# Fytex/Shafa-CD

Hardware: AMD Instinct MI355X
Metric: GiB/s Shannon-Fano encode+decode, 64 MiB blocks, 1/2/4/8 GPUs; bit-exact (higher is better)
Workload: dtype u8

## Files before the change

### shafa-cd_amd/csrc/sf_decode.hip

```cpp
#include <type_traits>
#include "common.hpp"
#include "internal.hpp"

#include <atomic>
#include <mutex>
#include <thread>

#include <algorithm>

#include <stdlib.h>

#include "sfd_common.hpp"
#include "sfd_dp.hpp"
#include "sfd_generic.hpp"

namespace {

typedef __attribute__((address_space(3))) u32 lds_u32;
typedef __attribute__((address_space(3))) u16 lds_u16;
typedef __attribute__((address_space(3))) u8 lds_u8;
template <int LONG> constexpr u32 spec_emask() { return LONG == 2 ? 31u : 15u; }

constexpr int SC_PHW = 16;
constexpr int SC_M = 4;
// ... 446 lines not shown
constexpr int SL_SW = 16;
constexpr int SL_ROW = SL_SW + 1;
constexpr int SL_STRIPS = DEC_THREADS + 1;
constexpr int SL_LDS_DATA = (SL_STRIPS * SL_ROW + 3) / 4 * 16;
constexpr int SL_MISC = DEC_THREADS + 16 + 32;

struct SlWin {
    u32 lo, hi, wa;
    __device__ __forceinline__ void init() { wa = 0xFFFFFFFFu; hi = lo = 0; }
    __device__ __forceinline__ u32 at(u32 q)
    {
        const u32 a = (q >> 3) & ~3u;
        if (a != wa) {
            const lds_u32 *pa = (const lds_u32 *)(size_t)a;
            lo = pa[0];
            hi = pa[1];
            wa = a;
        }
        return __builtin_amdgcn_alignbit(hi, lo, q);
    }
};

template <int LONG>
__device__ __forceinline__ void sl_walk(const lds_u8 *tab, const u16 *lt, const u32 KW, u32 &q, const u32 qe, const int qlimit, u32 &cnt, SlWin &sw)
{
    const u32 mask = (1u << KW) - 1u;
    auto long_len = [&](const u32 qq) -> u32 {
        const u32 win = __builtin_bitreverse32(sw.at(qq));
        const u32 l = (LONG == 1 ? long_code(lt, win) : long_code32(lt, win)) >> 8;
        return l ? l : 1u;
    };
    const u32 nlook = KW <= 10 ? 3u : 2u;
    while (q + nlook * KW <= qe && (int)(q + nlook * KW) <= qlimit) {
        const u32 w = sw.at(q);
        u32 sum = 0, e = 0;
        for (u32 i = 0; i < nlook; ++i) {
            e = tab[(w >> (sum & 31u)) & mask];
            sum += e;
        }
        q += sum & 31u;
        cnt += sum >> 5;
        if (LONG && __builtin_expect((e & 31u) == 0u, 0)) {
            const u32 l = long_len(q);
            if ((int)(q + l) > qlimit) { q = qe + spec_emask<LONG>(); return; }
            q += l;
            ++cnt;
        }
    }
    const lds_u8 *len0 = tab + (1u << KW);
    while (q < qe) {
        u32 l0 = len0[sw.at(q) & mask];
        if (LONG && __builtin_expect(l0 == 0u, 0)) l0 = long_len(q);
        if ((int)(q + l0) > qlimit) { q = qe + spec_emask<LONG>(); break; }
        q += l0;
        ++cnt;
    }
}

template <bool HAVE_OLD, int LONG>
__device__ __forceinline__ void sl_strip(const lds_u8 *tab, const u16 *lt, const u32 KW, const u32 qrow, const int qlimit, const u32 ent0,
                                         u32 (&ent)[2], u32 (&cnt)[2], u32 &exit_)
{
    u32 q = qrow + ent0;
    SlWin sw;
    sw.init();
#pragma unroll
    for (int k = 0; k < 2; ++k) {
        const u32 r = q - (qrow + 256u * k);
        if (HAVE_OLD && k > 0 && r == ent[k]) return;
        ent[k] = r;
        u32 c = 0;
        sl_walk<LONG>(tab, lt, KW, q, qrow + 256u * (k + 1), qlimit, c, sw);
        cnt[k] = c;
    }
    exit_ = (q - (qrow + 512u)) & spec_emask<LONG>();
}

template <int LONG>
__device__ __forceinline__ u32 sl_region(u8 *smem, const DecBlk &blk, const u32 tile0, const u32 e0_forced, u8 *__restrict__ chunk_entry,
                                         u16 *__restrict__ chunk_cnt, u32 *__restrict__ tile_cnt, u8 *__restrict__ tile_guess,
                                         u8 *__restrict__ tile_exit, const u32 tab_bytes)
{
    const u64 start = (u64)tile0 * DTILE;
    const u64 left = blk.in_n > start ? blk.in_n - start : 0;
    const size_t gt0 = (size_t)blk.tile_base + tile0;
    const u32 ntl = blk.n_tiles - tile0 < (u32)SC_WTILES ? blk.n_tiles - tile0 : (u32)SC_WTILES;
    u32 *data = (u32 *)smem;
    const u32 tab_off = SL_LDS_DATA;
    u8 *ex = smem + SL_LDS_DATA + tab_bytes;
    const u32 tid = threadIdx.x, lane = tid & 63, wv = tid >> 6;
    const u32 KW = blk.KW;
    const u16 *lt = (const u16 *)(smem + SL_LDS_DATA + tab_bytes + SL_MISC);
    {
        const long long base = (long long)start - 4 * SL_SW;
        constexpr u32 UNITS = (u32)(SL_STRIPS * SL_SW / 4 + 1), NIT = (UNITS + DEC_THREADS - 1) / DEC_THREADS;
        uint4 v[NIT];
#pragma unroll
        for (u32 it = 0; it < NIT; ++it) {
            const u32 i = tid + it * DEC_THREADS;
            const long long off = base + (long long)i * 16;
            v[it] = make_uint4(0, 0, 0, 0);
            if (i < UNITS && off >= 0 && (u64)off + 16 <= blk.in_n) v[it] = gload<uint4>(blk.in + off);
        }
#pragma unroll
        for (u32 it = 0; it < NIT; ++it) {
            const u32 i = tid + it * DEC_THREADS;
            if (i >= UNITS) break;
            const long long off = base + (long long)i * 16;
            u32 w[4] = {v[it].x, v[it].y, v[it].z, v[it].w};
            if (off >= 0 && (u64)off < blk.in_n && (u64)off + 16 > blk.in_n) {
                const int nv = (int)(blk.in_n - (u64)off);
#pragma unroll
                for (int q = 0; q < 16; ++q)
                    if (q < nv) w[q >> 2] |= (u32)gload<u8>(blk.in + off + q) << (8 * (q & 3));
            }
            const u32 f = 4 * i, at = f + f / SL_SW;
            const u32 w0 = rev_bytes(w[0]);
            if (f % SL_SW == 0 && f > 0) data[at - 1] = w0;
            if (i < UNITS - 1) {
                data[at] = w0;
                data[at + 1] = rev_bytes(w[1]);
                data[at + 2] = rev_bytes(w[2]);
                data[at + 3] = rev_bytes(w[3]);
            }
        }
    }
    __syncthreads();
    const int limit = (int)(left * 8) - (int)(512u * tid);
    const u32 qrow = 8u * ((4u * SL_ROW) * (tid + 1));
    const int qlimit = (int)qrow + limit;
    const lds_u8 *tab = (const lds_u8 *)(size_t)tab_off;
    u32 ent[2] = {0, 0}, cnt[2] = {0, 0}, exit_ = 0;
    {
        u32 e0;
        if (tid == 0) e0 = e0_forced;
        else {
            const u32 qe = qrow;
            u32 q = qe - 256u, dummy = 0;
            SlWin sw;
            sw.init();
            sl_walk<LONG>(tab, lt, KW, q, qe, qlimit, dummy, sw);
            e0 = (q - qe) & spec_emask<LONG>();
        }
        sl_strip<false, LONG>(tab, lt, KW, qrow, qlimit, e0, ent, cnt, exit_);
    }
    ex[tid] = (u8)exit_;
    __syncthreads();
    bool bad = false;
    u32 *const wsum = (u32 *)(ex + DEC_THREADS), *const flags = wsum + 4;
    u32 turn = 0;
    for (int round = 0; round < 4; ++round) {
        bad = tid > 0 && ent[0] != (u32)ex[tid - 1];
        if (!wg_any(bad, flags, turn)) break;
        if (bad) sl_strip<true, LONG>(tab, lt, KW, qrow, qlimit, (u32)ex[tid - 1], ent, cnt, exit_);
        __syncthreads();
        ex[tid] = (u8)exit_;
        __syncthreads();
        bad = tid > 0 && ent[0] != (u32)ex[tid - 1];
    }
    if (wg_any(bad, flags, turn)) {
        if (tid == 0) __hip_atomic_store(blk.run_dp, 1u, __ATOMIC_RELAXED, __HIP_MEMORY_SCOPE_AGENT);
    }
    const u32 my_tile = tid / 128u;
    const u32 wtot = dpp_scan_add(cnt[0] + cnt[1]);
    if (lane == 63) wsum[wv] = wtot;
    __syncthreads();
    if (my_tile < ntl) {
        const size_t c0 = gt0 * DEC_THREADS + (size_t)tid * 2;
        gstore<u16>(chunk_entry + c0, (u16)((ent[0] & 0xFFu) | (ent[1] << 8)));
        gstore<u32>(chunk_cnt + c0, cnt[0] | (cnt[1] << 16));
        const u32 in_tile = tid & 127u;
        if (in_tile == 0) {
            tile_cnt[gt0 + my_tile] = wsum[2 * my_tile] + wsum[2 * my_tile + 1];
            tile_guess[gt0 + my_tile] = (u8)ent[0];
        }
        if (in_tile == 127u) tile_exit[gt0 + my_tile] = (u8)exit_;
    }
    const u32 unit_exit = ex[ntl * 128u - 1u];
    __syncthreads();
    return unit_exit;
}

constexpr u32 SF_CHUNKS = 8;

constexpr u32 SF_LINKS = 2 * DEC_THREADS;
template <int LONG>
__device__ __forceinline__ void sf_links(u8 *smem, const DecBlk &blk, const u32 t_begin, const u32 t_end, u8 *__restrict__ chunk_entry,
                                         u16 *__restrict__ chunk_cnt, u32 *__restrict__ tile_cnt, u8 *__restrict__ tile_guess,
                                         const u8 *__restrict__ tile_exit, const u32 tab_bytes, const u32 long_bytes)
{
    const u32 tid = threadIdx.x, KW = blk.KW, mask = (1u << KW) - 1u;
    const u16 *lt = (const u16 *)(smem + tab_bytes + 48);
    const u8 *len0 = smem + (1u << KW);
    const u64 end_bit = blk.in_n * 8;
    u32 turn = 0;
    u32 xs[SF_LINKS / DEC_THREADS];
    bool any_bad = false;
#pragma unroll
    for (u32 i = 0; i < SF_LINKS / DEC_THREADS; ++i) {
        const u32 t = t_begin + tid + i * DEC_THREADS;
        xs[i] = 0xFFFFFFFFu;
        if (t < t_end) {
            const size_t gt = (size_t)blk.tile_base + t;
            const u32 x = tile_exit[gt - 1];
            if (tile_guess[gt] != x) { xs[i] = x; any_bad = true; }
        }
    }
    if (!wg_any(any_bad, (u32 *)(smem + tab_bytes), turn)) return;
    __syncthreads();
    fill_lds16((void *)smem, (const void *)blk.cnt3, 2u << KW);
    if (LONG) {
        const u16 *src = LONG == 1 ? blk.longtab : blk.long32;
        if (src) fill_lds16((void *)lt, src, long_bytes);
        else if (tid == 0) *(u16 *)lt = 0;
    }
    bool failed = false;
    volatile u32 *const gave_up = (volatile u32 *)(smem + tab_bytes + 32);
    if (tid == 0) *gave_up = 0;
    __syncthreads();
#pragma unroll 1
    for (u32 i = 0; i < SF_LINKS / DEC_THREADS; ++i) {
        if (*gave_up) break;
        const u32 x = xs[i];
        if (x == 0xFFFFFFFFu) continue;
        const u32 t = t_begin + tid + i * DEC_THREADS;
        const size_t gt = (size_t)blk.tile_base + t;
        const u64 tile_bit0 = (u64)t * DTILE * 8;
        if (x >= spec_emask<LONG>() || tile_bit0 + (u64)(SF_CHUNKS + 1) * CH_BITS + 64 > end_bit) { failed = true; *gave_up = 1; continue; }
        u32 q = x, wi = 0xFFFFFFFFu, lo = 0, hi = 0;
        auto window = [&](const u32 qq) -> u32 {
            const u32 i = qq >> 5;
            if (i != wi) {
                const u8 *p = blk.in + (u64)t * DTILE + 4u * i;
                lo = rev_bytes(gload<u32>(p));
                hi = rev_bytes(gload<u32>(p + 4));
                wi = i;
            }
            return __builtin_amdgcn_alignbit(hi, lo, qq);
        };
        int delta = 0;
        bool merged = false;
        const size_t c0 = gt * DEC_THREADS;
        for (u32 c = 0; c < SF_CHUNKS; ++c) {
            const u32 qe = CH_BITS * (c + 1);
            u32 cnt = 0;
            while (q < qe) {
                const u32 w = window(q);
                u32 l = len0[w & mask];
                if (LONG && l == 0u) {
                    const u32 win = __builtin_bitreverse32(w);
                    l = (LONG == 1 ? long_code(lt, win) : long_code32(lt, win)) >> 8;
                    if (!l) l = 1u;
                }
                q += l;
                ++cnt;
            }
            delta += (int)cnt - (int)chunk_cnt[c0 + c];
            chunk_cnt[c0 + c] = (u16)cnt;
            const u32 e = q - qe;
            if (e == (u32)chunk_entry[c0 + c + 1]) { merged = true; break; }
            chunk_entry[c0 + c + 1] = (u8)e;
        }
        if (!merged) { failed = true; *gave_up = 1; continue; }
        chunk_entry[c0] = (u8)x;
        tile_guess[gt] = (u8)x;
        tile_cnt[gt] = (u32)((int)tile_cnt[gt] + delta);
    }
    if (wg_any(failed, (u32 *)(smem + tab_bytes), turn) && tid == 0)
        __hip_atomic_store(blk.run_dp, 1u, __ATOMIC_RELAXED, __HIP_MEMORY_SCOPE_AGENT);
}

template <int LONG>
__global__ __launch_bounds__(DEC_THREADS) void sfd_ends(const DecBlk *__restrict__ blks, u8 *__restrict__ chunk_entry,
                                                        u16 *__restrict__ chunk_cnt, u32 *__restrict__ tile_cnt,
                                                        u8 *__restrict__ tile_guess, u8 *__restrict__ tile_exit, u32 tab_bytes, u32 long_bytes)
{
    extern __shared__ __attribute__((aligned(16))) u8 smem[];
    const DecBlk blk = blks[blockIdx.y];
    if (!blk.n_tiles || !blk.run_dp || __hip_atomic_load(blk.run_dp, __ATOMIC_RELAXED, __HIP_MEMORY_SCOPE_AGENT) != 0) return;
    if (lds_addr(smem) != 0) __builtin_trap();
    const u32 units = (blk.n_tiles + SC_WTILES - 1) / SC_WTILES;
    u32 first_end = units - 1;
    if (units >= 2 && blk.in_n - (u64)(units - 2) * SC_WTILES * DTILE < (u64)64 * SC_SB + 4) first_end = units - 2;
    if (blockIdx.x > 0) {
        const u32 t_end = first_end * SC_WTILES, t_begin = 1u + (blockIdx.x - 1u) * SF_LINKS;
        if (t_begin < t_end)
            sf_links<LONG>(smem, blk, t_begin, t_end, chunk_entry, chunk_cnt, tile_cnt, tile_guess, tile_exit, tab_bytes, long_bytes);
        return;
    }
    fill_lds16((void *)(smem + SL_LDS_DATA), (const void *)blk.cnt3, 2u << blk.KW);
    if (LONG) {
        u16 *lt = (u16 *)(smem + SL_LDS_DATA + tab_bytes + SL_MISC);
        const u16 *src = LONG == 1 ? blk.longtab : blk.long32;
        if (src) fill_lds16((void *)lt, src, long_bytes);
        else if (threadIdx.x == 0) *lt = 0;
    }
    __syncthreads();
    u32 e0 = first_end ? (u32)tile_exit[(size_t)blk.tile_base + first_end * SC_WTILES - 1] : 0u;
    for (u32 u = first_end; u < units; ++u)
        e0 = sl_region<LONG>(smem, blk, u * SC_WTILES, e0, chunk_entry, chunk_cnt, tile_cnt, tile_guess, tile_exit, tab_bytes);
}

constexpr int ws_row(bool esc) { return CH_BYTES / 4 + (esc ? 3 : 2); }
constexpr int ws_rows_bytes(bool esc)
{
    return 16 + (DEC_THREADS * ws_row(esc) + (esc ? 0 : DEC_THREADS / 16)) * 4;
}
constexpr int WS_MISC = 32;
typedef unsigned int u32x3_t __attribute__((ext_vector_type(3)));
constexpr u32 WS_NST = 4, WS_DROP = 0x7FFFFFF0u;
constexpr int WS_RSRC_FLAGS = 0x00020000, WS_AUX_NT = 2;

__device__ __forceinline__ void ws_walk1(const u32 tab_off, const u32 mask2, const u32 xa, u32 q2, const u32 q2end, u32 want,
                                         const bool by_pos)
{
    auto window2 = [&]() -> u32 {
        const lds_u32 *pa = (const lds_u32 *)(size_t)((q2 >> 3) & ~3u);
        return __builtin_amdgcn_alignbit(pa[1], pa[0], q2);
    };
    auto look = [&](const u32 w) -> u32 { return *(const lds_u16 *)(size_t)(tab_off + (w & mask2)); };
    auto image_or = [](const u32 at, const u32 v) {
        __hip_atomic_fetch_or((lds_u32 *)(size_t)at, v, __ATOMIC_RELAXED, __HIP_MEMORY_SCOPE_WORKGROUP);
    };
    if (by_pos) {
        constexpr u32 N = 3, F = 4, WPG = F * N / 4;
        const u32 s = (0u - xa) & 3u;
        u32 ptr = ((xa + 3u) & ~3u) - 4u;
        u32 L = 0, Lp = 0, Ep = 0;
        auto group = [&](auto first_group) -> bool {
            constexpr bool FIRST = decltype(first_group)::value;
            u32 x0 = 0, x1 = 0, ub = 0;
#pragma unroll
            for (u32 f = 0; f < F; ++f) {
                if (!((int)q2 < (int)q2end)) {
                    if (f == 0) {
                        if (!FIRST) {
                            image_or(ptr + 4u * (WPG - 1u), Ep);
                            image_or(ptr + 4u * WPG, __builtin_amdgcn_alignbyte(0u, Lp, s));
                        }
                    } else {
                        const u32 at = ptr + 4u * (f * N >> 2);
                        image_or(at, __builtin_amdgcn_alignbyte(L, Lp, s));
                        image_or(at + 4u, __builtin_amdgcn_alignbyte(0u, L, s));
                    }
                    return false;
                }
                if (f == 0 && !FIRST) {
                    *(lds_u32 *)(size_t)(ptr + 4u * (WPG - 1u)) = Ep;
                    ptr += 4u * WPG;
                }
                u32 w;
                if ((f & 1u) == 0) {
                    const lds_u32 *pa = (const lds_u32 *)(size_t)((q2 >> 3) & ~3u);
                    const u32 w0 = pa[0], w1 = pa[1], w2 = pa[2];
                    w = x0 = __builtin_amdgcn_alignbit(w1, w0, q2);
                    x1 = __builtin_amdgcn_alignbit(w2, w1, q2);
                } else
                    w = __builtin_amdgcn_alignbit(x1, x0, ub);
                u32 ua = 0;
#pragma unroll
                for (u32 i = 0; i < N; ++i) {
                    const u32 k = f * N + i, b = k & 3u;
                    const u32 e = look(w >> ua);
                    ua += e >> 8;
                    L = __builtin_amdgcn_perm(e, L, b == 0 ? 0x0C0C0C04u : b == 1 ? 0x0C0C0400u : b == 2 ? 0x0C040100u : 0x04020100u);
                    if (b == 3u) {
                        const u32 E = __builtin_amdgcn_alignbyte(L, Lp, s), at = ptr + 4u * (k >> 2);
                        Lp = L;
                        if (FIRST && k == 3u) image_or(at, E);
                        else if (k == F * N - 1u) Ep = E;
                        else *(lds_u32 *)(size_t)at = E;
                    }
                }
                q2 += ua;
                ub = ua;
            }
            return true;
        };
        if (group(std::true_type{}))
            while (group(std::false_type{})) {}
        return;
    }
    u32 wp = xa & ~3u, nb = 8u * (xa & 3u), acc = 0;
    for (; want; --want) {
        const u32 e = look(window2());
        q2 += e >> 8;
        acc |= (e & 0xFFu) << nb;
        nb += 8u;
        if (nb == 32u) {
            image_or(wp, acc);
            wp += 4u;
            acc = nb = 0;
        }
    }
    if (nb) image_or(wp, acc);
}

template <int LONG, bool ESC, bool ONE = false>
__global__ __launch_bounds__(DEC_THREADS) void sfd_wstage(const DecBlk *__restrict__ blks, const u8 *__restrict__ chunk_entry,
                                                          const u16 *__restrict__ chunk_cnt, const u64 *__restrict__ tile_off,
                                                          u32 tpw, u32 tab_bytes, u32 cap, u32 long_bytes)
{
    extern __shared__ __attribute__((aligned(16))) u8 smem[];
    const DecBlk blk = blks[blockIdx.y];
    const u32 first_tile = blockIdx.x * tpw;
    if (first_tile >= blk.n_tiles) return;
    if (tile_off[(size_t)blk.tile_base + first_tile] >= blk.n_sym) return;
    const u32 LONGB = LONG ? long_bytes : 0u;
    u32 *rows = (u32 *)(smem + 16);
    constexpr u32 WS_ROW = (u32)ws_row(ESC), tab_off = (u32)ws_rows_bytes(ESC);
    const u16 *lt = (const u16 *)(smem + tab_off + tab_bytes);
    const u32 img_off = tab_off + tab_bytes + LONGB;
    u32 *wsum = (u32 *)(smem + img_off + cap);
    u32 *next = wsum + 4;
    const u32 tid = threadIdx.x, lane = tid & 63, wv = tid >> 6;
    const u32 K1 = blk.K1, K3 = sym3_window(K1);
    const u32 sh = 32 - K1;
    static_assert(!ONE || (LONG == 0 && !ESC), "the one-code walk has no escapes");
    constexpr bool one = ONE;
    fill_lds16(smem + tab_off, (const void *)blk.sym3, (one ? 2u : 4u) << K3);
    if (LONG) {
        const u16 *src = LONG == 1 ? blk.longtab : blk.long32;
        if (src) fill_lds16((void *)lt, src, LONGB);
        else if (tid == 0) *(u16 *)lt = 0;
    }
    for (u32 i = tid; i < cap / 16; i += DEC_THREADS) *(uint4 *)(smem + img_off + 16 * i) = make_uint4(0, 0, 0, 0);
    bool bad = false;
    if (lds_addr(smem) != 0) __builtin_trap();
    const u32 q2row = 8u * (16u + 4u * (WS_ROW * tid + (ESC ? 0u : tid >> 4))) - (one ? 1u : 2u);
    const u32 mask4 = ((1u << K3) - 1u) << (one ? 1 : 2);
    auto fetch16 = [&](const u64 off) -> uint4 {
        if (off + 16 <= blk.in_n) return gload_nt<uint4>(blk.in + off);
        u32 w[4] = {0, 0, 0, 0};
        if (off < blk.in_n) {
            const int nv = (int)(blk.in_n - off);
#pragma unroll
            for (int q = 0; q < 16; ++q)
                if (q < nv) w[q >> 2] |= (u32)gload<u8>(blk.in + off + q) << (8 * (q & 3));
        }
        return make_uint4(w[0], w[1], w[2], w[3]);
    };
    uint4 pf0, pf1;
    u32 pf2[ESC ? 3 : 2] = {};
    auto fetch_ahead = [&](const u64 off) {
        constexpr int NB = ESC ? 12 : 8;
        if (off + NB <= blk.in_n) {
            if constexpr (ESC) {
                const u32x3_t v = __builtin_nontemporal_load((const GLOBAL_AS u32x3_t *)(unsigned long long)(blk.in + off));
                pf2[0] = v.x; pf2[1] = v.y; pf2[2] = v.z;
            } else {
                const uint2 v = gload_nt<uint2>(blk.in + off);
                pf2[0] = v.x; pf2[1] = v.y;
            }
            return;
        }
        u32 w[3] = {0, 0, 0};
        if (off < blk.in_n) {
            const int nv = (int)(blk.in_n - off);
#pragma unroll
            for (int q = 0; q < NB; ++q)
                if (q < nv) w[q >> 2] |= (u32)gload<u8>(blk.in + off + q) << (8 * (q & 3));
        }
#pragma unroll
        for (int q = 0; q < NB / 4; ++q) pf2[q] = w[q];
    };
    u8 pf_entry = 0, pf_next = 0;
    u16 pf_cnt = 0;
    auto prefetch = [&](const u32 tile) {
        const u64 base = (u64)tile * DTILE;
        const size_t g = ((size_t)blk.tile_base + tile) * DEC_THREADS + tid;
        pf_entry = chunk_entry[g];
        pf_cnt = chunk_cnt[g];
        pf_next = (tile + 1 < blk.n_tiles || tid + 1 < (u32)DEC_THREADS) ? chunk_entry[g + 1] : (u8)0;
        pf0 = fetch16(base + 16ull * tid);
        pf1 = fetch16(base + 16ull * (tid + DEC_THREADS));
        if (tid == 0) fetch_ahead(base + DTILE);
    };
    auto put16 = [&](const u32 i, const uint4 v) {
        const u32 f = 4 * i, at = f + (WS_ROW - 8u) * (f >> 3) + (ESC ? 0u : f >> 7);
        const u32 w0 = rev_bytes(v.x), w1 = rev_bytes(v.y), w2 = rev_bytes(v.z);
        if ((f & 7u) == 0 && f > 0) {
            const u32 lk = at - (WS_ROW - 8u) - (!ESC && (f & 127u) == 0 ? 1u : 0u);
            rows[lk] = w0;
            rows[lk + 1] = w1;
            if (ESC) rows[lk + 2] = w2;
        }
        if (i < (u32)(DTILE / 16)) {
            rows[at] = w0;
            rows[at + 1] = w1;
            rows[at + 2] = w2;
            rows[at + 3] = rev_bytes(v.w);
        }
    };
    auto store_bytes = [&](u8 *ga, const uint4 v, const u32 lo, const u32 hi) {
        const u32 wds[4] = {v.x, v.y, v.z, v.w};
#pragma unroll
        for (u32 q = 0; q < 16; ++q)
            if (q >= lo && q < hi) gstore<u8>(ga + q, (u8)(wds[q >> 2] >> (8 * (q & 3))));
    };
    u32 carry_n = 0, carry_lo = 0;
    u8 *carry_g = nullptr;
    prefetch(first_tile);
    __builtin_amdgcn_s_waitcnt(0x0F70);
    for (u32 it = 0; it < tpw; ++it) {
        const u32 tile = first_tile + it;
        if (tile >= blk.n_tiles) break;
        const size_t gt = (size_t)blk.tile_base + tile;
        const u64 toff = tile_off[gt];
        if (toff >= blk.n_sym) break;
        lds_barrier();
        put16(tid, pf0);
        put16(tid + DEC_THREADS, pf1);
        if (tid == 0) put16(DTILE / 16, make_uint4(pf2[0], pf2[1], ESC ? pf2[ESC ? 2 : 0] : 0u, 0u));
        const u32 entry = pf_entry, cnt = pf_cnt, nent = pf_next;
        if (it + 1 < tpw && tile + 1 < blk.n_tiles) prefetch(tile + 1);
        const u32 incl = wave_incl_scan_add<u32>(cnt);
        if (lane == 63) wsum[wv] = incl;
        lds_barrier();
        u32 pre = incl - cnt, total = 0;
        for (u32 w = 0; w < 4; ++w) { if (w < wv) pre += wsum[w]; total += wsum[w]; }
        const u64 room = blk.n_sym - toff;
        const u32 tot_c = (u32)__builtin_amdgcn_readfirstlane((int)(room < (u64)total ? (u32)room : total));
        u32 want = pre >= tot_c ? 0u : (tot_c - pre < cnt ? tot_c - pre : cnt);
        u32 q2 = q2row + entry;
        const bool by_pos = want == cnt && tile + 1 < blk.n_tiles && nent != spec_emask<LONG>();
        const u32 q2end = q2row + 256u + nent;
        u32 done = 0;
        do {
            u8 *gout = blk.out + toff + done;
            const u32 mis = (u32)((uintptr_t)gout & 15u);
            if (carry_g && (carry_n != mis || carry_g != gout - mis)) {
                if (tid == 0) {
                    uint4 *ip = (uint4 *)(smem + img_off);
                    store_bytes(carry_g, *ip, carry_lo, carry_n);
                    ip[0] = make_uint4(0, 0, 0, 0);
                    ip[1] = make_uint4(0, 0, 0, 0);
                }
                carry_n = 0;
                carry_g = nullptr;
                lds_barrier();
            }
            const u32 capw = cap - 32;
            u32 nxt = tot_c;
            if (mis + (tot_c - done) > capw) {
                if (tid == 0) *next = tot_c;
                lds_barrier();
                if (want && pre >= done && mis + (pre - done) + want > capw) atomicMin(next, pre);
                lds_barrier();
                nxt = (u32)__builtin_amdgcn_readfirstlane((int)*next);
                lds_barrier();
            }
            const bool mine = want && pre >= done && pre + want <= nxt;
            if constexpr (ONE) {
                if (mine) ws_walk1(tab_off, mask4, img_off + mis + (pre - done), q2, q2end, want, by_pos);
            } else if (mine) {
                const u32 x = mis + (pre - done);
                u32 wp = img_off + (x & ~3u), nbx = x << 30, acc = 0;
                auto emit = [&](const u32 e) {
                    const u32 sh = nbx >> 27, syms = e & 0xFFFFFFu;
                    acc |= syms << sh;
                    if (__builtin_add_overflow(nbx, e & 0xC0000000u, &nbx)) {
                        __hip_atomic_fetch_or((lds_u32 *)(size_t)wp, acc, __ATOMIC_RELAXED, __HIP_MEMORY_SCOPE_WORKGROUP);
                        wp += 4u;
                        acc = syms >> (32u - sh);
                    }
                };
                auto window4 = [&]() -> u32 {
                    const lds_u32 *pa = (const lds_u32 *)(size_t)((q2 >> 3) & ~3u);
                    return __builtin_amdgcn_alignbit(pa[1], pa[0], q2);
                };
                auto step = [&](const bool tail) {
                    u32 e = *(const lds_u32 *)(size_t)(tab_off + (window4() & mask4));
                    if (ESC && __builtin_expect((e >> 30) == 0, 0)) {
                        const u32 q = q2 + 2u;
                        const lds_u32 *pb = (const lds_u32 *)(size_t)((q >> 3) & ~3u);
                        const u32 win = __builtin_bitreverse32(__builtin_amdgcn_alignbit(pb[1], pb[0], q));
                        u32 e1 = LONG == 1 ? long_code(lt, win) : LONG == 2 ? long_code32(lt, win)
                                           : (u32)gload<u16>(blk.lut13 + (win >> sh));
                        if (e1 == 0) { bad = true; e1 = 1u << 8; }
                        e = (e1 & 0xFFu) | ((e1 >> 8) << 24) | (1u << 30);
                    }
                    u32 n = e >> 30, syms = e & 0xFFFFFFu;
                    if (tail) {
                        n = n < want ? n : want;
                        syms &= (1u << (8 * n)) - 1u;
                    }
                    emit(syms | n << 30);
                    q2 += (e >> 24) & 63u;
                    want -= n;
                };
                auto multi = [&](auto nlook) {
                    constexpr u32 N = decltype(nlook)::value;
                    if (by_pos) {
                        while ((int)q2 < (int)q2end) {
                            const u32 w4 = window4();
                            u32 ua = 0, e = 0;
#pragma unroll
                            for (u32 i = 0; i < N; ++i) {
                                e = *(const lds_u32 *)(size_t)(tab_off + ((w4 >> (ua & 31u)) & mask4));
                                emit(e);
                                ua += e >> 24;
                            }
                            q2 += ua & 63u;
                            if (ESC && __builtin_expect((e >> 30) == 0, 0)) step(false);
                        }
                        want = 0;
                    }
                    while (want >= 3 * N) {
                        const u32 w4 = window4();
                        u32 ua = 0, e = 0;
#pragma unroll
                        for (u32 i = 0; i < N; ++i) {
                            e = *(const lds_u32 *)(size_t)(tab_off + ((w4 >> (ua & 31u)) & mask4));
                            emit(e);
                            ua += e >> 24;
                        }
                        q2 += ua & 63u;
                        want -= ua >> 6;
                        if (ESC && __builtin_expect((e >> 30) == 0, 0)) step(false);
                    }
                };
                if (K3 <= 10) multi(std::integral_constant<u32, 3>{});
                else if (K3 <= 15) multi(std::integral_constant<u32, 2>{});
                while (want) step(true);
                if (nbx) __hip_atomic_fetch_or((lds_u32 *)(size_t)wp, acc, __ATOMIC_RELAXED, __HIP_MEMORY_SCOPE_WORKGROUP);
            }
            lds_barrier();
            const u32 end = mis + (nxt - done);
            const u32 lo0 = (carry_n == mis && carry_n) ? carry_lo : mis;
            const u32 nfull = end >> 4;
            u8 *const g0 = gout - mis;
            if constexpr (LONG == 2) {
                for (u32 u = tid; u < nfull; u += DEC_THREADS) {
                    uint4 *ip = (uint4 *)(smem + img_off + 16 * u);
                    const uint4 v = *ip;
                    *ip = make_uint4(0, 0, 0, 0);
                    if (u == 0 && lo0) store_bytes(g0, v, lo0, 16u);
                    else gstore_nt<uint4>(g0 + 16 * u, v);
                }
            } else {
                const __amdgpu_buffer_rsrc_t win = __builtin_amdgcn_make_buffer_rsrc(g0, 0, (int)(16u * nfull), WS_RSRC_FLAGS);
                u32 ub = tid;
                do {
#pragma unroll
                    for (u32 s = 0; s < WS_NST; ++s) {
                        const u32 u = ub + s * DEC_THREADS;
                        u32x4_t x = {0u, 0u, 0u, 0u};
                        u32 off = WS_DROP;
                        if (u < nfull) {
                            uint4 *ip = (uint4 *)(smem + img_off + 16 * u);
                            const uint4 v = *ip;
                            *ip = make_uint4(0, 0, 0, 0);
                            if (s == 0 && u == 0 && lo0) store_bytes(g0, v, lo0, 16u);
                            else {
                                x.x = v.x; x.y = v.y; x.z = v.z; x.w = v.w;
                                off = 16u * u;
                            }
                        }
                        __builtin_amdgcn_raw_buffer_store_b128(x, win, (int)off, 0, WS_AUX_NT);
                    }
                    ub += WS_NST * DEC_THREADS;
                } while (__builtin_amdgcn_readfirstlane((int)(ub - tid)) < (int)nfull);
            }
            if (tid == 0 && nfull) {
                uint4 *ip = (uint4 *)(smem + img_off);
                const uint4 a = ip[nfull], b = ip[nfull + 1];
                ip[nfull] = make_uint4(0, 0, 0, 0);
                ip[nfull + 1] = make_uint4(0, 0, 0, 0);
                ip[0] = a;
                ip[1] = b;
            }
            carry_lo = nfull ? 0u : lo0;
            carry_n = end & 15u;
            carry_g = g0 + 16 * nfull;
            done = nxt;
            if (done < tot_c) lds_barrier();
        } while (done < tot_c);
    }
    if (tid == 0 && carry_n) {
        const uint4 v = *(const uint4 *)(smem + img_off);
        store_bytes(carry_g, v, carry_lo, carry_n);
    }
    if (bad) set_error(blk.err, SHAFA_FILE_UNRECOGNIZABLE);
}

__global__ __launch_bounds__(DEC_THREADS) void sfd_offsets(const DecBlk *__restrict__ blks,
                                                           const u32 *__restrict__ tile_cnt, u64 *__restrict__ tile_off)
{
    __shared__ u64 wtot[4];
    __shared__ u64 carry;
    const DecBlk blk = blks[blockIdx.x];
    const u32 tid = threadIdx.x, lane = tid & 63, wv = tid >> 6;
    if (tid == 0) carry = 0;
    __syncthreads();
    constexpr u32 OFF_EPT = 16;
    for (u32 r0 = 0; r0 < blk.n_tiles; r0 += DEC_THREADS * OFF_EPT) {
        const u32 t0 = r0 + tid * OFF_EPT;
        u32 x[OFF_EPT];
#pragma unroll
        for (u32 j = 0; j < OFF_EPT; ++j) x[j] = t0 + j < blk.n_tiles ? tile_cnt[blk.tile_base + t0 + j] : 0u;
        u64 mine = 0;
#pragma unroll
        for (u32 j = 0; j < OFF_EPT; ++j) mine += x[j];
        const u64 incl = wave_incl_scan_add<u64>(mine);
        if (lane == 63) wtot[wv] = incl;
        __syncthreads();
        u64 base = carry + incl - mine;
        for (u32 w = 0; w < wv; ++w) base += wtot[w];
#pragma unroll
        for (u32 j = 0; j < OFF_EPT; ++j) {
            if (t0 + j < blk.n_tiles) tile_off[blk.tile_base + t0 + j] = base;
            base += x[j];
        }
        __syncthreads();
        if (tid == 0) carry += wtot[0] + wtot[1] + wtot[2] + wtot[3];
        __syncthreads();
    }
    if (tid == 0 && carry < blk.n_sym) set_error(blk.err, SHAFA_FILE_UNRECOGNIZABLE);
}

}

#include "sfd_host_tables.hpp"

template <class F> static void for_blocks_parallel(int nblocks, F fn)
{
    std::atomic<int> next{0};
    auto work = [&]() {
        for (;;) {
            const int b = next.fetch_add(1, std::memory_order_relaxed);
            if (b >= nblocks) break;
            fn(b);
        }
    };
    int helpers = nblocks / 16;
    const int hw = (int)std::thread::hardware_concurrency();
    if (helpers > 7) helpers = 7;
    if (hw > 0 && helpers > hw - 1) helpers = hw - 1;
    std::vector<std::thread> th;
    for (int i = 0; i < helpers; ++i) {
        try { th.emplace_back(work); } catch (...) { break; }
    }
    work();
    for (auto &t : th) t.join();
}

static int g_sfd_speculate = 1;
void sfdec_configure(int speculate) { g_sfd_speculate = speculate; }
static int g_sfd_path = 0;
void sfdec_configure_path(int path) { g_sfd_path = path; }

static bool spec_worthwhile(const shafa_code_table &t, const HostTab &h, bool force)
{
    if (!h.ok || !(h.complete || h.complete16 || h.complete32) || h.lmax > 32 || h.lmax < 2) return false;
    if (force) return true;
    const u64 key = spec_key(t.len, t.bits);
    static u64 ckey[1024];
    static signed char cval[1024];
    static std::mutex cmu;
    const u32 slot = (u32)(key >> 17) & 1023u;
    {
        std::lock_guard<std::mutex> lk(cmu);
        if (cval[slot] && ckey[slot] == key) return cval[slot] == 2;
    }
    u64 rs = key | 1ull;
    int fails = 0;
    for (int trial = 0; trial < SPEC_TRIALS && fails <= SPEC_MAX_FAILS; ++trial) {
        u64 w[SPEC_WORDS];
        for (u64 &x : w) x = spec_rand(rs);
        if (!spec_trial(w, h.lenlut.data(), h.K1)) ++fails;
    }
    const bool yes = fails <= SPEC_MAX_FAILS;
    std::lock_guard<std::mutex> lk(cmu);
    ckey[slot] = key;
    cval[slot] = yes ? 2 : 1;
    return yes;
}

struct SfdArrays {
    u8 *cfn, *tfn;
    u8 *tent, *cent;
    u16 *ccnt;
    u32 *tcnt;
    u64 *toff;
    u8 *tguess, *texit;
};

enum SfdForm { SFD_MID32, SFD_LONG_ALL, SFD_PACKED12, SFD_PACKED13, SFD_PACKED };

static u32 sfd_tpw(u32 most, u32 max_tiles, int nblocks)
{
    u32 tpw = most;
    while (tpw > 1 && (u64)ceil_div_u64(max_tiles, tpw) * nblocks < 2048) tpw >>= 1;
    return tpw;
}

static void sfd_launch_packed(hipStream_t st, const DecBlk *dblk, int nblocks, u32 max_tiles, SfdForm form, bool esc, bool spec,
                              u32 tabb, u32 long_used, bool all_spec, u32 ws_tab, u32 ws_cap, const SfdArrays &a, bool one = false)
{
    static decltype(&sfd_scan<0>) const scans[3] = {sfd_scan<2>, sfd_scan<1>, sfd_scan<0>};
    static decltype(&sfd_ends<0>) const ends[3] = {sfd_ends<2>, sfd_ends<1>, sfd_ends<0>};
    static decltype(&sfd_sync16<true, false>) const syncs[4] = {sfd_sync16<false, true>, sfd_sync16<true, false, 12>,
                                                                sfd_sync16<true, false, 13>, sfd_sync16<true, false>};
    const int f = form < SFD_PACKED12 ? form : 2;
    const dim3 grid_b((u32)nblocks), wg(DEC_THREADS);
    hipLaunchKernelGGL(sfd_tables, dim3((u32)nblocks, 8), wg, 0, st, dblk);
    if (spec) {
        const size_t lds_scan = (size_t)SC_LDS_ROWS + tabb + SC_MISC + long_used;
        const size_t lds_ends = (size_t)SL_LDS_DATA + tabb + SL_MISC + long_used;
        hipLaunchKernelGGL(scans[f], dim3((u32)ceil_div_u64(max_tiles, SC_TILES), (u32)nblocks), wg, lds_scan, st, dblk, a.cent, a.ccnt,
                           a.tcnt, a.tguess, a.texit, tabb, long_used);
        hipLaunchKernelGGL(ends[f], dim3(1u + (u32)ceil_div_u64(max_tiles, SF_LINKS), (u32)nblocks), wg, lds_ends, st, dblk, a.cent,
                           a.ccnt, a.tcnt, a.tguess, a.texit, tabb, long_used);
    }
    const u32 tpw = all_spec ? 256u : sfd_tpw(4, max_tiles, nblocks);
    const dim3 grid_f((u32)ceil_div_u64(max_tiles, tpw), (u32)nblocks);
    if (form == SFD_MID32) {
        hipLaunchKernelGGL(sfd_sync32, grid_f, wg, 0, st, dblk, a.cfn, a.tfn, tpw);
        hipLaunchKernelGGL(sfd_tiles, grid_b, wg, (size_t)32 * DEC_THREADS + DEC_THREADS, st, dblk, 32u, (const u8 *)a.tfn, a.tent);
        hipLaunchKernelGGL(sfd_countfsm32, grid_f, wg, 0, st, dblk, (const u8 *)a.cfn, (const u8 *)a.tent, a.cent, a.ccnt, a.tcnt, tpw);
    } else {
        constexpr int CSUBS = 4;
        hipLaunchKernelGGL(syncs[form - SFD_LONG_ALL], grid_f, wg, 0, st, dblk, (u64 *)a.cfn, (u64 *)a.tfn, tpw);
        hipLaunchKernelGGL(sfd_tiles16, grid_b, wg, 0, st, dblk, (const u64 *)a.tfn, a.tent);
        hipLaunchKernelGGL((sfd_countfsm<CSUBS>), dim3((u32)ceil_div_u64(max_tiles, tpw * CSUBS), (u32)nblocks), dim3(DEC_THREADS * CSUBS),
                           0, st, dblk, (const u64 *)a.cfn, (const u8 *)a.tent, a.cent, a.ccnt, a.tcnt, tpw);
    }
    hipLaunchKernelGGL(sfd_offsets, grid_b, wg, 0, st, dblk, (const u32 *)a.tcnt, a.toff);
    static decltype(&sfd_wstage<0, false>) const wstages[5] = {sfd_wstage<2, true>, sfd_wstage<1, true>, sfd_wstage<0, true>,
                                                               sfd_wstage<0, false>, sfd_wstage<0, false, true>};
    const u32 tpw_ws = sfd_tpw(16, max_tiles, nblocks);
    const size_t lds_ws = (size_t)ws_rows_bytes(esc) + ws_tab + ws_cap + WS_MISC + long_used;
    hipLaunchKernelGGL(wstages[one ? 4 : f == 2 && !esc ? 3 : f], dim3((u32)ceil_div_u64(max_tiles, tpw_ws), (u32)nblocks), wg, lds_ws, st,
                       dblk, (const u8 *)a.cent, (const u16 *)a.ccnt, (const u64 *)a.toff, tpw_ws, ws_tab, ws_cap, long_used);
}

static int sfd_launch_bytemap(hipStream_t st, const DecBlk *dblk, u32 nb, u32 max_tiles, u32 R, u32 l2cap, const SfdArrays &a)
{
    const size_t lds_lut = (size_t)(1u << LUT_MAXK) * 2 + (size_t)l2cap * 2;
    const size_t lds_sync = (size_t)LDS_DATA + (size_t)R * DEC_THREADS + lds_lut + 4 * R + 64;
    const size_t lds_count = lds_sync + DEC_THREADS;
    const size_t lds_write = (size_t)LDS_DATA + lds_lut + 64;
    const size_t lds_tiles = (size_t)R * DEC_THREADS + DEC_THREADS;
    if (lds_tiles > 65536 || lds_sync > 65536) {
        HIP_TRY(hipFuncSetAttribute((const void *)sfd_sync, hipFuncAttributeMaxDynamicSharedMemorySize, (int)lds_sync));
        HIP_TRY(hipFuncSetAttribute((const void *)sfd_count, hipFuncAttributeMaxDynamicSharedMemorySize, (int)lds_count));
        HIP_TRY(hipFuncSetAttribute((const void *)sfd_tiles, hipFuncAttributeMaxDynamicSharedMemorySize, (int)lds_tiles));
    }
    const dim3 grid_t(max_tiles, nb), grid_b(nb), wg(DEC_THREADS);
    hipLaunchKernelGGL(sfd_sync, grid_t, wg, lds_sync, st, dblk, R, l2cap, a.cfn, a.tfn);
    hipLaunchKernelGGL(sfd_tiles, grid_b, wg, lds_tiles, st, dblk, R, (const u8 *)a.tfn, a.tent);
    hipLaunchKernelGGL(sfd_count, grid_t, wg, lds_count, st, dblk, R, l2cap, (const u8 *)a.cfn, (const u8 *)a.tent, a.cent, a.ccnt,
                       a.tcnt);
    hipLaunchKernelGGL(sfd_offsets, grid_b, wg, 0, st, dblk, (const u32 *)a.tcnt, a.toff);
    hipLaunchKernelGGL(sfd_write, grid_t, wg, lds_write, st, dblk, l2cap, (const u8 *)a.cent, (const u16 *)a.ccnt, (const u64 *)a.toff);
    return SHAFA_SUCCESS;
}

int sfdec_launch(Batch *bt, hipStream_t st, int nblocks, const u8 *d_in, const u64 *h_in_off,
                 const u64 *h_in_n, const shafa_code_table *h_tables, const u64 *h_n_symbols, u8 *d_out,
                 const u64 *h_out_off)
{
    if (nblocks <= 0) return SHAFA_SUCCESS;
    if (nblocks > bt->max_blocks) return SHAFA_LACK_OF_MEMORY;

    std::vector<HostTab> tabs(nblocks);
    u32 lmax_all = 1, max_tiles = 0, max_l2 = 0;
    u64 total_tiles = 0;
    size_t tab_bytes = 0;
    std::vector<u32> ntiles(nblocks, 0);
    bool pair_all = true;
    bool c16_all = true;
    bool c32_all = true;
    for (int b = 0; b < nblocks; ++b)
        if ((h_in_off[b] & 15) || (h_out_off[b] & 15)) return SHAFA_OUTSIDE_MODULE;
    {
        std::atomic<bool> nomem{false};
        for_blocks_parallel(nblocks, [&](int b) {
            try { build_host_tab(h_tables[b], tabs[b]); } catch (...) { nomem.store(true); }
        });
        if (nomem.load()) return SHAFA_LACK_OF_MEMORY;
    }
    for (int b = 0; b < nblocks; ++b) {
        HostTab &h = tabs[b];
        bool run = h_n_symbols[b] > 0;
        if (run && (!h.ok || h.empty)) {
            bt->h_hosterr[b] = SHAFA_FILE_UNRECOGNIZABLE;
            run = false;
        }
        if (run && h_in_n[b] == 0) { bt->h_hosterr[b] = SHAFA_FILE_UNRECOGNIZABLE; run = false; }
        if (!run) continue;
        ntiles[b] = (u32)ceil_div_u64(h_in_n[b], DTILE);
        total_tiles += ntiles[b];
        if (ntiles[b] > max_tiles) max_tiles = ntiles[b];
        if (h.lmax > lmax_all) lmax_all = h.lmax;
        tab_bytes += ((h.lut.size() * 2 + 15) & ~(size_t)15) + ((h.trie.size() * 4 + 15) & ~(size_t)15) +
                     ((h.lenlut.size() + 15) & ~(size_t)15) + ((h.lut2.size() * 2 + 16 + 15) & ~(size_t)15) +
                     ((h.lut13.size() * 2 + 15) & ~(size_t)15) + (h.longtab.empty() ? 0 : (size_t)LONG_BYTES) +
                     (h.long32.empty() ? 0 : (size_t)((LONG32_BYTES + 15) & ~15)) + ((h.lenlut32.size() + 15) & ~(size_t)15);
        if (h.lut2.size() > max_l2) max_l2 = (u32)h.lut2.size();
        pair_all = pair_all && h.complete;
        c16_all = c16_all && h.complete16;
        c32_all = c32_all && (h.complete16 || h.complete32);
    }
    if (!total_tiles) return SHAFA_SUCCESS;
    u32 R = 16;
    while (R < lmax_all) R <<= 1;
    if (g_sfd_path >= 1) pair_all = c16_all = c32_all = false;
    const bool long_all = R == 16 && !pair_all && c16_all && lmax_all > (u32)LEN_MAXK;
    const bool packed = R == 16 && ((pair_all && lmax_all <= (u32)LEN_MAXK) || long_all);
    const bool mid32 = !packed && R == 32 && c32_all;
    const bool ws_esc = mid32 || long_all || lmax_all > (u32)SYM3_MAXK;
    bool ws_one = !ws_esc;
    for (int b = 0; b < nblocks; ++b)
        if (ntiles[b] && !tabs[b].one) ws_one = false;
    if (!packed && !mid32 && R < 32) R = 32;

    size_t off = 0;
    const size_t o_blk = off; off += ((size_t)nblocks * sizeof(DecBlk) + 15) & ~(size_t)15;
    const size_t o_rundp = off; off += ((size_t)nblocks * 4 + 15) & ~(size_t)15;
    const size_t o_tab = off; off += tab_bytes;
    const size_t stage_bytes = off;
    const size_t o_tilefn = off; off += (size_t)total_tiles * (R < 8 ? 8 : R); off = (off + 15) & ~(size_t)15;
    const size_t o_tent = off; off += (size_t)total_tiles; off = (off + 15) & ~(size_t)15;
    const size_t o_tcnt = off; off += (size_t)total_tiles * 4; off = (off + 15) & ~(size_t)15;
    const size_t o_toff = off; off += (size_t)total_tiles * 8;
    const size_t o_cent = off; off += (size_t)total_tiles * DEC_THREADS; off = (off + 15) & ~(size_t)15;
    const size_t o_ccnt = off; off += (size_t)total_tiles * DEC_THREADS * 2; off = (off + 15) & ~(size_t)15;
    const bool need_tabs = packed || mid32;
    const size_t o_pair = off; off += (packed && pair_all) ? (size_t)nblocks * (2u << LEN_MAXK) : 0;
    const size_t o_cnt3 = off; off += need_tabs ? (size_t)nblocks * (2u << LEN_MAXK) : 0;
    const size_t o_sym3 = off; off += need_tabs ? (size_t)nblocks * (4u << LEN_MAXK) : 0;
    const size_t o_fsm4 = off; off += need_tabs ? (size_t)nblocks * 16384 : 0;
    const size_t o_fsm1 = off; off += need_tabs ? (size_t)nblocks * 2048 : 0;
    const size_t o_cfn = off; off += packed ? (size_t)total_tiles * DEC_THREADS * 8 : (size_t)total_tiles * R * DEC_THREADS;
    const bool spec_path = (packed || mid32) && g_sfd_speculate != 0;
    std::vector<u32> hblk_kw(nblocks, 0);
    for (int b = 0; b < nblocks; ++b) {
        if (!ntiles[b]) continue;
        u32 n13 = 0;
        if (tabs[b].K1 == 13)
            for (int sy = 0; sy < 256; ++sy) n13 += h_tables[b].len[sy] == 13;
        hblk_kw[b] = scan_window(tabs[b].K1, long_all || mid32, n13);
    }
    u32 long_used = 0;
    if (long_all) {
        u32 gmax = 0;
        for (int b = 0; b < nblocks; ++b)
            if (ntiles[b] && !tabs[b].longtab.empty() && tabs[b].longtab[0] > gmax) gmax = tabs[b].longtab[0];
        long_used = (16u + (u32)LONG_PFX * 2u + gmax * 32u + 15u) & ~15u;
    } else if (mid32) {
        u32 nmax = 0;
        for (int b = 0; b < nblocks; ++b)
            if (ntiles[b] && !tabs[b].long32.empty() && tabs[b].long32[1] > nmax) nmax = tabs[b].long32[1];
        long_used = (16u + (u32)LONG_PFX * 4u + nmax * 4u + 15u) & ~15u;
    }
    std::vector<char> spec_blk(nblocks, 0);
    bool any_spec = false;
    for (int b = 0; spec_path && b < nblocks; ++b)
        if (ntiles[b] && spec_worthwhile(h_tables[b], tabs[b], g_sfd_speculate == 2)) { spec_blk[b] = 1; any_spec = true; }
    const size_t o_tguess = off; off += any_spec ? (size_t)total_tiles : 0; off = (off + 15) & ~(size_t)15;
    const size_t o_texit = off; off += any_spec ? (size_t)total_tiles : 0; off = (off + 15) & ~(size_t)15;
    int rc = batch_reserve(bt, st, off);
    if (rc) return rc;
    u8 *ws = (u8 *)bt->d_ws;

    u8 *dpar = batch_params_begin(bt, stage_bytes);
    if (!dpar) return SHAFA_LACK_OF_MEMORY;
    ParamsScope pscope(bt, st);
    u8 *hs = (u8 *)batch_stage(bt, bt->par_inline ? st : bt->copy_st, stage_bytes);
    if (!hs) return SHAFA_LACK_OF_MEMORY;
    DecBlk *hb = (DecBlk *)hs;
    size_t tpos = o_tab;
    u32 tbase = 0;
    std::vector<size_t> tab_pos(nblocks, 0);
    for (int b = 0; b < nblocks; ++b) {
        DecBlk &e = hb[b];
        memset(&e, 0, sizeof(e));
        e.in = d_in + h_in_off[b];
        e.out = d_out + h_out_off[b];
        e.in_n = h_in_n[b];
        e.n_sym = h_n_symbols[b];
        e.err = bt->d_err + b;
        e.n_tiles = ntiles[b];
        e.tile_base = tbase;
        e.run_dp = any_spec ? (u32 *)(dpar + o_rundp) + b : nullptr;
        ((u32 *)(hs + o_rundp))[b] = spec_blk[b] ? 0u : 1u;
        e.pairlut = (packed && pair_all) ? ws + o_pair + (size_t)b * (2u << LEN_MAXK) : nullptr;
        e.cnt3 = need_tabs ? (u16 *)(ws + o_cnt3 + (size_t)b * (2u << LEN_MAXK)) : nullptr;
        e.sym3 = need_tabs ? (u32 *)(ws + o_sym3 + (size_t)b * (4u << LEN_MAXK)) : nullptr;
        e.fsm4 = need_tabs ? (u32 *)(ws + o_fsm4 + (size_t)b * 16384) : nullptr;
        e.fsm1 = need_tabs ? (u32 *)(ws + o_fsm1 + (size_t)b * 2048) : nullptr;
        tbase += ntiles[b];
        if (!ntiles[b]) continue;
        HostTab &h = tabs[b];
        e.K = h.K;
        e.K1 = h.K1;
        e.KW = hblk_kw[b];
        e.lmax = h.lmax;
        e.one = ws_one;
        e.n_states = (u32)(h.trie.size() / 2);
        tab_pos[b] = tpos;
        e.lut2 = (const u16 *)(dpar + tpos);
        e.n_l2 = (u32)h.lut2.size();
        tpos += (h.lut2.size() * 2 + 16 + 15) & ~(size_t)15;
        e.lut13 = (const u16 *)(dpar + tpos);
        tpos += (h.lut13.size() * 2 + 15) & ~(size_t)15;
        if (!h.longtab.empty()) {
            e.longtab = (const u16 *)(dpar + tpos);
            tpos += LONG_BYTES;
        }
        if (!h.long32.empty()) {
            e.long32 = (const u16 *)(dpar + tpos);
            tpos += (LONG32_BYTES + 15) & ~15;
        }
        if (!h.lenlut32.empty()) {
            e.lenlut32 = dpar + tpos;
            tpos += (h.lenlut32.size() + 15) & ~(size_t)15;
        }
        e.lenlut = dpar + tpos;
        if (!e.lenlut32) e.lenlut32 = e.lenlut;
        tpos += (h.lenlut.size() + 15) & ~(size_t)15;
        e.lut = (const u16 *)(dpar + tpos);
        tpos += (h.lut.size() * 2 + 15) & ~(size_t)15;
        e.trie = (const u32 *)(dpar + tpos);
        tpos += (h.trie.size() * 4 + 15) & ~(size_t)15;
    }
    for_blocks_parallel(nblocks, [&](int b) {
        if (!ntiles[b]) return;
        const HostTab &h = tabs[b];
        size_t q = tab_pos[b];
        if (h.lut2.size()) memcpy(hs + q, h.lut2.data(), h.lut2.size() * 2);
        q += (h.lut2.size() * 2 + 16 + 15) & ~(size_t)15;
        memcpy(hs + q, h.lut13.data(), h.lut13.size() * 2);
        q += (h.lut13.size() * 2 + 15) & ~(size_t)15;
        if (!h.longtab.empty()) { memcpy(hs + q, h.longtab.data(), LONG_BYTES); q += LONG_BYTES; }
        if (!h.long32.empty()) { memcpy(hs + q, h.long32.data(), LONG32_BYTES); q += (LONG32_BYTES + 15) & ~15; }
        if (!h.lenlut32.empty()) { memcpy(hs + q, h.lenlut32.data(), h.lenlut32.size()); q += (h.lenlut32.size() + 15) & ~(size_t)15; }
        memcpy(hs + q, h.lenlut.data(), h.lenlut.size());
        q += (h.lenlut.size() + 15) & ~(size_t)15;
        memcpy(hs + q, h.lut.data(), h.lut.size() * 2);
        q += (h.lut.size() * 2 + 15) & ~(size_t)15;
        memcpy(hs + q, h.trie.data(), h.trie.size() * 4);
    });
    if ((rc = batch_params_commit(bt, st, hs, stage_bytes))) return rc;

    const DecBlk *dblk = (const DecBlk *)(dpar + o_blk);
    const SfdArrays arr = {ws + o_cfn, ws + o_tilefn, ws + o_tent, ws + o_cent, (u16 *)(ws + o_ccnt), (u32 *)(ws + o_tcnt),
                           (u64 *)(ws + o_toff), ws + o_tguess, ws + o_texit};
    if (!packed && !mid32) {
        if ((rc = sfd_launch_bytemap(st, dblk, (u32)nblocks, max_tiles, R, (max_l2 + 8) & ~7u, arr))) return rc;
        HIP_TRY(hipGetLastError());
        return pscope.done();
    }
    u32 k1_max = 1, k1_all = 0;
    bool all_spec = any_spec;
    for (int b = 0; b < nblocks; ++b) {
        if (!ntiles[b]) continue;
        if (spec_blk[b] && hblk_kw[b] > k1_max) k1_max = hblk_kw[b];
        k1_all = (k1_all == 0 || k1_all == tabs[b].K1) ? tabs[b].K1 : 0xFFFFFFFFu;
        if (!spec_blk[b]) all_spec = false;
    }
    const SfdForm form = mid32 ? SFD_MID32 : long_all ? SFD_LONG_ALL : k1_all == 12 ? SFD_PACKED12 : k1_all == 13 ? SFD_PACKED13
                                                                                                          : SFD_PACKED;
    u32 ws_tab = 16;
    for (int b = 0; b < nblocks; ++b) {
        const u32 k3 = sym3_window(tabs[b].K1), tb = (ws_one ? 2u : 4u) << k3;
        if (tb > ws_tab) ws_tab = tb;
    }
    u32 ws_cap = 4096, ws_tight = 4096;
    for (int b = 0; b < nblocks; ++b) {
        if (!ntiles[b]) continue;
        const u64 per_tile = ceil_div_u64(h_n_symbols[b], ntiles[b]);
        const u64 c = per_tile + per_tile / 8 + 1024, t = per_tile + per_tile / 32 + 256;
        if (c > ws_cap) ws_cap = (u32)(c > 40960 ? 40960 : c);
        if (t > ws_tight) ws_tight = (u32)(t > 40960 ? 40960 : t);
    }
    {
        const u32 base = (u32)ws_rows_bytes(ws_esc) + ws_tab + long_used + (u32)WS_MISC;
        const u32 most = 65536u - base;
        if (ws_cap > most) ws_cap = most;
        constexpr u32 steps[3] = {20480u, 26880u, 40960u};
        for (u32 k = 0; k < 3; ++k) {
            if (base + ((ws_tight + 15u) & ~15u) <= steps[k]) {
                ws_cap = steps[k] - base;
                if (ws_cap > most) ws_cap = most;
                break;
            }
        }
    }
    ws_cap &= ~15u;
    sfd_launch_packed(st, dblk, nblocks, max_tiles, form, ws_esc, any_spec, 2u << k1_max, long_used, all_spec, ws_tab, ws_cap, arr, ws_one);
    HIP_TRY(hipGetLastError());
    return pscope.done();
}

#include "sfd_dev.hpp"
```

Measured before the change: 875.9.

## Store one-code walk input in column-major LDS planes to avoid bank conflicts

For the one-code decode walk, each thread's input chunk is now stored as interleaved word columns (one plane per word index across threads) instead of per-thread rows. Each thread's bitstream words then sit in distinct LDS banks, so its 2-3 word window reads become strided plane reads that do not conflict. The lookup table moves to offset 0, and the slot in front of each column is reused. This adds layout-specific address math and compile-time bank and bijection checks, and the launch falls back when the table or capacity is too small.

Result: faster. 889.2, median of 4 (+1.5%).

```diff
diff --git a/shafa-cd_amd/csrc/sf_decode.hip b/shafa-cd_amd/csrc/sf_decode.hip
--- a/shafa-cd_amd/csrc/sf_decode.hip
+++ b/shafa-cd_amd/csrc/sf_decode.hip
@@ -772,21 +772,89 @@
 }
 
 constexpr int ws_row(bool esc) { return CH_BYTES / 4 + (esc ? 3 : 2); }
-constexpr int ws_rows_bytes(bool esc)
-{
-    return 16 + (DEC_THREADS * ws_row(esc) + (esc ? 0 : DEC_THREADS / 16)) * 4;
+struct WsCols {
+    static constexpr u32 PLANE = 4u * DEC_THREADS;
+    static constexpr u32 WORDS = CH_BYTES / 4 + 2;
+    static constexpr u32 BYTES = WORDS * PLANE;
+    static constexpr u32 TAB_MIN = PLANE;
+    static constexpr u32 Q0 = 31u;
+    static constexpr u32 word_at(u32 f) { return (f & 7u) * DEC_THREADS + (f >> 3); }
+    static constexpr u32 ahead_at(u32 f) { return (8u + (f & 7u)) * DEC_THREADS + (f >> 3) - 1u; }
+    u32 col0;
+    __device__ __forceinline__ u32 front(const u32 tid) const { return col0 - PLANE + 4u * tid; }
+    static __device__ __forceinline__ u32 word_of_bit(const u32 cf, const u32 q)
+    {
+        u32 a;
+        asm("v_lshl_add_u32 %0, %1, 10, %2" : "=v"(a) : "v"(q >> 5), "v"(cf));
+        return a;
+    }
+    static __device__ __forceinline__ u32 word(const u32 a, const u32 j) { return *(const lds_u32 *)(size_t)(a + j * PLANE); }
+    __device__ __forceinline__ void put16(const u32 i, const uint4 v) const
+    {
+        const u32 f = 4u * i, w0 = rev_bytes(v.x), w1 = rev_bytes(v.y);
+        if ((i & 1u) == 0 && i > 0) {
+            const u32 lk = col0 + 4u * ahead_at(f);
+            *(lds_u32 *)(size_t)lk = w0;
+            *(lds_u32 *)(size_t)(lk + PLANE) = w1;
+        }
+        if (i < (u32)(DTILE / 16)) {
+            const u32 at = col0 + 4u * word_at(f);
+            *(lds_u32 *)(size_t)at = w0;
+            *(lds_u32 *)(size_t)(at + PLANE) = w1;
+            *(lds_u32 *)(size_t)(at + 2u * PLANE) = rev_bytes(v.z);
+            *(lds_u32 *)(size_t)(at + 3u * PLANE) = rev_bytes(v.w);
+        }
+    }
+    static constexpr bool banks_ok()
+    {
+        for (u32 i = 0; i < WORDS; ++i)
+            for (u32 c0 = 0; c0 < (u32)DEC_THREADS; c0 += 32) {
+                u32 seen = 0;
+                for (u32 c = c0; c < c0 + 32; ++c) seen |= 1u << ((i * DEC_THREADS + c) & 31u);
+                if (seen != 0xFFFFFFFFu) return false;
+            }
+        return true;
+    }
+    static constexpr bool bijection_ok()
+    {
+        bool seen[DTILE / 4] = {};
+        for (u32 f = 0; f < (u32)(DTILE / 4); ++f) {
+            const u32 d = word_at(f);
+            if (d >= (u32)(DTILE / 4) || seen[d] || d % DEC_THREADS != f / 8 || d / DEC_THREADS != f % 8) return false;
+            seen[d] = true;
+        }
+        return true;
+    }
+    static constexpr bool ahead_ok()
+    {
+        for (u32 c = 0; c < (u32)DEC_THREADS; ++c)
+            for (u32 k = 0; k < 2; ++k)
+                if (ahead_at(8u * (c + 1u) + k) != (8u + k) * DEC_THREADS + c || word_at(8u * (c + 1u) + k) != k * DEC_THREADS + c + 1u)
+                    return false;
+        return true;
+    }
+    static constexpr u32 last_word_read(u32 max_entry) { return ((Q0 + CH_BITS + max_entry - 1u) >> 5) + 2u; }
+};
+static_assert(WsCols::PLANE == 1024 && WsCols::BYTES == 10240, "ds_read2st64_b32 steps in units of 256 bytes: offsets 0 and 4");
+static_assert(WsCols::banks_ok() && WsCols::bijection_ok() && WsCols::ahead_ok(), "the column layout of the one-code walk");
+static_assert((WsCols::last_word_read(spec_emask<0>()) - 1u) * WsCols::PLANE + 4u * DEC_THREADS <= WsCols::BYTES + WsCols::PLANE,
+              "the walk's third word lies at most one plane behind the columns (in the image)");
+static_assert(WsCols::TAB_MIN >= WsCols::PLANE && (WsCols::Q0 >> 5) == 0, "the word in front of a column lies in the table's slot");
+constexpr int ws_rows_bytes(bool esc, bool one = false)
+{
+    return one ? (int)WsCols::BYTES : 16 + (DEC_THREADS * ws_row(esc) + (esc ? 0 : DEC_THREADS / 16)) * 4;
 }
 constexpr int WS_MISC = 32;
 typedef unsigned int u32x3_t __attribute__((ext_vector_type(3)));
 constexpr u32 WS_NST = 4, WS_DROP = 0x7FFFFFF0u;
 constexpr int WS_RSRC_FLAGS = 0x00020000, WS_AUX_NT = 2;
 
-__device__ __forceinline__ void ws_walk1(const u32 tab_off, const u32 mask2, const u32 xa, u32 q2, const u32 q2end, u32 want,
-                                         const bool by_pos)
+__device__ __forceinline__ void ws_walk1(const u32 tab_off, const u32 mask2, const u32 cf, const u32 xa, u32 q2, const u32 q2end,
+                                         u32 want, const bool by_pos)
 {
     auto window2 = [&]() -> u32 {
-        const lds_u32 *pa = (const lds_u32 *)(size_t)((q2 >> 3) & ~3u);
-        return __builtin_amdgcn_alignbit(pa[1], pa[0], q2);
+        const u32 pa = WsCols::word_of_bit(cf, q2);
+        return __builtin_amdgcn_alignbit(WsCols::word(pa, 1), WsCols::word(pa, 0), q2);
     };
     auto look = [&](const u32 w) -> u32 { return *(const lds_u16 *)(size_t)(tab_off + (w & mask2)); };
     auto image_or = [](const u32 at, const u32 v) {
@@ -821,8 +889,8 @@
                 }
                 u32 w;
                 if ((f & 1u) == 0) {
-                    const lds_u32 *pa = (const lds_u32 *)(size_t)((q2 >> 3) & ~3u);
-                    const u32 w0 = pa[0], w1 = pa[1], w2 = pa[2];
+                    const u32 pa = WsCols::word_of_bit(cf, q2);
+                    const u32 w0 = WsCols::word(pa, 0), w1 = WsCols::word(pa, 1), w2 = WsCols::word(pa, 2);
                     w = x0 = __builtin_amdgcn_alignbit(w1, w0, q2);
                     x1 = __builtin_amdgcn_alignbit(w2, w1, q2);
                 } else
@@ -878,9 +946,10 @@
     if (tile_off[(size_t)blk.tile_base + first_tile] >= blk.n_sym) return;
     const u32 LONGB = LONG ? long_bytes : 0u;
     u32 *rows = (u32 *)(smem + 16);
-    constexpr u32 WS_ROW = (u32)ws_row(ESC), tab_off = (u32)ws_rows_bytes(ESC);
+    constexpr u32 WS_ROW = (u32)ws_row(ESC), tab_off = ONE ? 0u : (u32)ws_rows_bytes(ESC);
+    const WsCols cols{tab_bytes};
     const u16 *lt = (const u16 *)(smem + tab_off + tab_bytes);
-    const u32 img_off = tab_off + tab_bytes + LONGB;
+    const u32 img_off = (ONE ? tab_bytes + WsCols::BYTES : tab_off + tab_bytes) + LONGB;
     u32 *wsum = (u32 *)(smem + img_off + cap);
     u32 *next = wsum + 4;
     const u32 tid = threadIdx.x, lane = tid & 63, wv = tid >> 6;
@@ -897,7 +966,7 @@
     for (u32 i = tid; i < cap / 16; i += DEC_THREADS) *(uint4 *)(smem + img_off + 16 * i) = make_uint4(0, 0, 0, 0);
     bool bad = false;
     if (lds_addr(smem) != 0) __builtin_trap();
-    const u32 q2row = 8u * (16u + 4u * (WS_ROW * tid + (ESC ? 0u : tid >> 4))) - (one ? 1u : 2u);
+    const u32 q2row = ONE ? WsCols::Q0 : 8u * (16u + 4u * (WS_ROW * tid + (ESC ? 0u : tid >> 4))) - 2u;
     const u32 mask4 = ((1u << K3) - 1u) << (one ? 1 : 2);
     auto fetch16 = [&](const u64 off) -> uint4 {
         if (off + 16 <= blk.in_n) return gload_nt<uint4>(blk.in + off);
@@ -947,6 +1016,7 @@
         if (tid == 0) fetch_ahead(base + DTILE);
     };
     auto put16 = [&](const u32 i, const uint4 v) {
+        if constexpr (ONE) { cols.put16(i, v); return; }
         const u32 f = 4 * i, at = f + (WS_ROW - 8u) * (f >> 3) + (ESC ? 0u : f >> 7);
         const u32 w0 = rev_bytes(v.x), w1 = rev_bytes(v.y), w2 = rev_bytes(v.z);
         if ((f & 7u) == 0 && f > 0) {
@@ -1022,7 +1092,7 @@
             }
             const bool mine = want && pre >= done && pre + want <= nxt;
             if constexpr (ONE) {
-                if (mine) ws_walk1(tab_off, mask4, img_off + mis + (pre - done), q2, q2end, want, by_pos);
+                if (mine) ws_walk1(tab_off, mask4, cols.front(tid), img_off + mis + (pre - done), q2, q2end, want, by_pos);
             } else if (mine) {
                 const u32 x = mis + (pre - done);
                 u32 wp = img_off + (x & ~3u), nbx = x << 30, acc = 0;
@@ -1300,7 +1370,7 @@
     static decltype(&sfd_wstage<0, false>) const wstages[5] = {sfd_wstage<2, true>, sfd_wstage<1, true>, sfd_wstage<0, true>,
                                                                sfd_wstage<0, false>, sfd_wstage<0, false, true>};
     const u32 tpw_ws = sfd_tpw(16, max_tiles, nblocks);
-    const size_t lds_ws = (size_t)ws_rows_bytes(esc) + ws_tab + ws_cap + WS_MISC + long_used;
+    const size_t lds_ws = (size_t)ws_rows_bytes(esc, one) + ws_tab + ws_cap + WS_MISC + long_used;
     hipLaunchKernelGGL(wstages[one ? 4 : f == 2 && !esc ? 3 : f], dim3((u32)ceil_div_u64(max_tiles, tpw_ws), (u32)nblocks), wg, lds_ws, st,
                        dblk, (const u8 *)a.cent, (const u16 *)a.ccnt, (const u64 *)a.toff, tpw_ws, ws_tab, ws_cap, long_used);
 }
@@ -1533,7 +1603,7 @@
     }
     const SfdForm form = mid32 ? SFD_MID32 : long_all ? SFD_LONG_ALL : k1_all == 12 ? SFD_PACKED12 : k1_all == 13 ? SFD_PACKED13
                                                                                                           : SFD_PACKED;
-    u32 ws_tab = 16;
+    u32 ws_tab = ws_one ? WsCols::TAB_MIN : 16u;
     for (int b = 0; b < nblocks; ++b) {
         const u32 k3 = sym3_window(tabs[b].K1), tb = (ws_one ? 2u : 4u) << k3;
         if (tb > ws_tab) ws_tab = tb;
@@ -1547,7 +1617,7 @@
         if (t > ws_tight) ws_tight = (u32)(t > 40960 ? 40960 : t);
     }
     {
-        const u32 base = (u32)ws_rows_bytes(ws_esc) + ws_tab + long_used + (u32)WS_MISC;
+        const u32 base = (u32)ws_rows_bytes(ws_esc, ws_one) + ws_tab + long_used + (u32)WS_MISC;
         const u32 most = 65536u - base;
         if (ws_cap > most) ws_cap = most;
         constexpr u32 steps[3] = {20480u, 26880u, 40960u};
@@ -1560,6 +1630,7 @@
         }
     }
     ws_cap &= ~15u;
+    if (ws_one && (ws_tab < WsCols::TAB_MIN || ws_cap < WsCols::PLANE)) return SHAFA_OUTSIDE_MODULE;
     sfd_launch_packed(st, dblk, nblocks, max_tiles, form, ws_esc, any_spec, 2u << k1_max, long_used, all_spec, ws_tab, ws_cap, arr, ws_one);
     HIP_TRY(hipGetLastError());
     return pscope.done();
```
